# chasewalker26/Image-Classification-XAI

Measured on AMD Instinct MI355X. Metric: attributions/sec (IG 50-step ResNet-50 224^2), higher is better.
Workload: dtype f32

## Files before the change

image-classification-xai_amd/csrc/conv/conv1x1_bwd_wide_kernels.hip:

```cpp
#include "xai_common.h"
#include "xai_conv_walk.h"
#include "xai_convw.h"

XAI_VERSION_ENTRIES(xai_convw_version, XAI_CONVW_VERSION, XAI_CONVW_MINOR)

namespace {

typedef float f32x4 __attribute__((ext_vector_type(4)));

__device__ __forceinline__ f32x4 mfma4(float a, float b, f32x4 c) { return __builtin_amdgcn_mfma_f32_16x16x4f32(a, b, c, 0, 0, 0); }

__global__ __launch_bounds__(kWave) void conv1x1_bwd_wide_simple_kernel(const float* __restrict__ gy, const float* __restrict__ W, int K,
                                                                        int C, int HW, int grouping, int from_zero, XaiStagger st,
                                                                        float* __restrict__ gx) {
  const int lane = threadIdx.x, slot = lane >> 4, l16 = lane & 15;
  const int row = blockIdx.y * 16 + l16;
  const int col = blockIdx.x * 16 + l16;
  const bool row_ok = row < C, col_ok = col < HW;
  const float* gyn = gy + static_cast<int64_t>(blockIdx.z) * K * HW + (col_ok ? col : 0);
  float* gxn = gx + static_cast<int64_t>(blockIdx.z) * C * HW + (col_ok ? col : 0);
  const int first = xai_stagger_first(st, 16 * (st.axis == XAI_STAGGER_ROWS ? blockIdx.y : blockIdx.x));
  f32x4 acc = {0.f, 0.f, 0.f, 0.f};
  for (int t = 0; t < st.blocks; ++t) {
    const int k0 = xai_stagger_block(st, first, t) * kWalkBlock;
#pragma unroll
    for (int m = 0; m < 4; ++m) {
      const int k = k0 + xai_walk_k(grouping, m, slot);
      const float a = row_ok ? W[static_cast<int64_t>(k) * C + row] : 0.f;
      const float b = col_ok ? gyn[static_cast<int64_t>(k) * HW] : 0.f;
      acc = mfma4(a, b, acc);
    }
  }
  if (from_zero) acc = f32x4{0.f, 0.f, 0.f, 0.f} + acc;
  if (!col_ok) return;
#pragma unroll
  for (int r = 0; r < 4; ++r) {
    const int c = blockIdx.y * 16 + 4 * slot + r;
    if (c < C) gxn[static_cast<int64_t>(c) * HW] = acc[r];
  }
}

constexpr int kThreads = 256;
constexpr int kPad = 16;

__device__ __forceinline__ f32x4 load4(const float* p, int valid, bool vec) {
  f32x4 v = {0.f, 0.f, 0.f, 0.f};
  if (valid <= 0) return v;
  if (vec) return *reinterpret_cast<const f32x4*>(p);
#pragma unroll
  for (int j = 0; j < 4; ++j)
    if (j < valid) v[j] = p[j];
  return v;
}

template <int TM, int TN>
__global__ __launch_bounds__(kThreads) void conv1x1_bwd_wide_kernel(const float* __restrict__ gy, const float* __restrict__ W, int K, int C,
                                                                    int HW, int grouping, int from_zero, XaiStagger st, int hold, int vec,
                                                                    float* __restrict__ gx) {
  constexpr int LDA = TM + kPad, LDB = TN + kPad;
  constexpr int WROWS = TM / 32, WCOLS = 4 / WROWS, NJ = TN / (16 * WCOLS);
  constexpr int UA = TM / 4, UB = TN / 4;
  constexpr int RA = kWalkBlock * UA / kThreads;
  static_assert(RA >= 1 && kWalkBlock * UB <= kThreads && NJ >= 1, "tile sizes");
  extern __shared__ __attribute__((aligned(16))) float lds[];
  float* As = lds;
  float* Bs = lds + 2 * kWalkBlock * LDA;
  const int tid = threadIdx.x, lane = tid & (kWave - 1), wave = tid / kWave;
  const int slot = lane >> 4, l16 = lane & 15;
  const int col0 = blockIdx.x * TN, n = blockIdx.y;
  const int nb = st.blocks;
  const int chunks = hold ? (C + TM - 1) / TM : 1, chunk0 = hold ? 0 : blockIdx.z;
  const int first = xai_stagger_first(st, col0);

  const int bk = tid / UB, bj = (tid % UB) * 4;
  const bool b_lane = tid < kWalkBlock * UB;
  const int b_valid = b_lane ? min(4, HW - (col0 + bj)) : 0;
  const float* bp = gy + static_cast<int64_t>(n) * K * HW + (b_valid > 0 ? col0 + bj : 0);
  f32x4 ra[RA], rb;
  auto load = [&](int g) {
    const int chunk = chunk0 + g / nb, block = xai_stagger_block(st, first, g % nb);
    const int k0 = block * kWalkBlock;
#pragma unroll
    for (int r = 0; r < RA; ++r) {
      const int u = tid + r * kThreads, ak = u / UA, ai = chunk * TM + (u % UA) * 4;
      ra[r] = load4(W + static_cast<int64_t>(k0 + ak) * C + (ai < C ? ai : 0), C - ai, vec != 0);
    }
    if (g < nb || !hold) rb = load4(bp + static_cast<int64_t>(k0 + bk) * HW, b_valid, vec != 0);
  };
  auto stage = [&](int g) {
    float* A = As + (g & 1) * kWalkBlock * LDA;
#pragma unroll
    for (int r = 0; r < RA; ++r) {
      const int u = tid + r * kThreads, ak = u / UA, ai = (u % UA) * 4;
      *reinterpret_cast<f32x4*>(A + xai_walk_row(grouping, ak) * LDA + ai) = ra[r];
    }
    if (b_lane && (g < nb || !hold)) {
      float* B = Bs + (hold ? xai_stagger_block(st, first, g % nb) : (g & 1)) * kWalkBlock * LDB;
      *reinterpret_cast<f32x4*>(B + xai_walk_row(grouping, bk) * LDB + bj) = rb;
    }
  };

  const int wr = (wave / WCOLS) * 32, wc = (wave % WCOLS) * (16 * NJ);
  f32x4 acc[2][NJ];
#pragma unroll
  for (int i = 0; i < 2; ++i)
#pragma unroll
    for (int j = 0; j < NJ; ++j) acc[i][j] = f32x4{0.f, 0.f, 0.f, 0.f};

  const int slabs = chunks * nb;
  load(0);
  stage(0);
  __syncthreads();
  int t = 0;
  for (int g = 0; g < slabs; ++g) {
    const bool more = g + 1 < slabs;
    if (more) load(g + 1);
    const float* A = As + (g & 1) * kWalkBlock * LDA;
    const float* B = Bs + (hold ? xai_stagger_block(st, first, t) : (g & 1)) * kWalkBlock * LDB;
#pragma unroll
    for (int m = 0; m < 4; ++m) {
      const int krow = 4 * m + slot;
      const float a0 = A[krow * LDA + wr + l16], a1 = A[krow * LDA + wr + 16 + l16];
      float b[NJ];
#pragma unroll
      for (int j = 0; j < NJ; ++j) b[j] = B[krow * LDB + wc + 16 * j + l16];
#pragma unroll
      for (int j = 0; j < NJ; ++j) {
        acc[0][j] = mfma4(a0, b[j], acc[0][j]);
        acc[1][j] = mfma4(a1, b[j], acc[1][j]);
      }
    }
    if (more) stage(g + 1);
    __syncthreads();
    if (++t < nb) continue;
    t = 0;
    const int row0 = (chunk0 + g / nb) * TM;
#pragma unroll
    for (int j = 0; j < NJ; ++j) {
      const int col = col0 + wc + 16 * j + l16;
      float* out = gx + static_cast<int64_t>(n) * C * HW + col;
#pragma unroll
      for (int i = 0; i < 2; ++i) {
        if (from_zero) acc[i][j] = f32x4{0.f, 0.f, 0.f, 0.f} + acc[i][j];
#pragma unroll
        for (int r = 0; r < 4; ++r) {
          const int c = row0 + wr + 16 * i + 4 * slot + r;
          if (col < HW && c < C) out[static_cast<int64_t>(c) * HW] = acc[i][j][r];
        }
        acc[i][j] = f32x4{0.f, 0.f, 0.f, 0.f};
      }
    }
  }
}

constexpr int kHoldBytes = 40 * 1024;

static int wide_args_status(const float* gy, const float* weight, int N, int K, int C, int HW, int grouping, int depth, int tile, int axis,
                            int stagger, int stride, const float* gx, XaiStagger* st) {
  XAI_REQUIRE_PTR(gy); XAI_REQUIRE_PTR(weight); XAI_REQUIRE_PTR(gx);
  XAI_REQUIRE(N > 0 && K > 0 && C > 0 && HW > 0, XAI_E_SHAPE);
  XAI_REQUIRE(((reinterpret_cast<uintptr_t>(gy) | reinterpret_cast<uintptr_t>(weight) | reinterpret_cast<uintptr_t>(gx)) & 3u) == 0,
              XAI_E_SHAPE);
  XAI_REQUIRE(grouping == XAI_WALK_K_CONSECUTIVE || grouping == XAI_WALK_K_STRIDE4, XAI_E_SHAPE);
  XAI_REQUIRE(xai_stagger_plan(K, depth, tile, axis, stagger, stride, st), XAI_E_SHAPE);
  XAI_REQUIRE(N <= 65535 && static_cast<int64_t>(K) * HW <= INT32_MAX && static_cast<int64_t>(C) * HW <= INT32_MAX, XAI_E_UNSUPPORTED);
  return XAI_OK;
}

}

XAI_EXPORT int xai_convw_bwd_data_f32(const float* gy, const float* weight, int N, int K, int C, int HW, int grouping, int from_zero,
                                      int depth, int tile, int axis, int stagger, int stride, float* gx, xai_stream_t stream) {
  XaiStagger st;
  if (const int rc = wide_args_status(gy, weight, N, K, C, HW, grouping, depth, tile, axis, stagger, stride, gx, &st)) return rc;
  XAI_REQUIRE(st.mask == 0 || (axis == XAI_STAGGER_COLUMNS && tile % 32 == 0), XAI_E_UNSUPPORTED);
  const int tn = st.mask != 0 && tile % 64 != 0 ? 32 : 64, tm = C <= 64 ? 64 : 128;
  const int chunks = static_cast<int>(xai_ceil_div(C, tm));
  const size_t slab_b = sizeof(float) * kWalkBlock * (tn + kPad);
  const bool hold = chunks > 1 && slab_b * st.blocks <= static_cast<size_t>(kHoldBytes);
  XAI_REQUIRE(chunks <= 65535, XAI_E_UNSUPPORTED);
  const bool vec = HW % 4 == 0 && C % 4 == 0 && xai_aligned16(gy) && xai_aligned16(weight);
  const size_t lds = sizeof(float) * 2 * kWalkBlock * (tm + kPad) + slab_b * (hold ? st.blocks : 2);
  const dim3 grid(static_cast<unsigned>(xai_ceil_div(HW, tn)), static_cast<unsigned>(N), static_cast<unsigned>(hold ? 1 : chunks));
  hipStream_t s = static_cast<hipStream_t>(stream);
  xai_dispatch(tm == 128, [&](auto tall) {
    xai_dispatch(tn == 64, [&](auto broad) {
      constexpr int TM = decltype(tall)::value ? 128 : 64, TN = decltype(broad)::value ? 64 : 32;
      hipLaunchKernelGGL((conv1x1_bwd_wide_kernel<TM, TN>), grid, dim3(kThreads), lds, s, gy, weight, K, C, HW, grouping, from_zero != 0, st,
                         hold ? 1 : 0, vec ? 1 : 0, gx);
    });
  });
  return xai_launch_status();
}

XAI_EXPORT int xai_convw_bwd_data_simple_f32(const float* gy, const float* weight, int N, int K, int C, int HW, int grouping, int from_zero,
                                             int depth, int tile, int axis, int stagger, int stride, float* gx, xai_stream_t stream) {
  XaiStagger st;
  if (const int rc = wide_args_status(gy, weight, N, K, C, HW, grouping, depth, tile, axis, stagger, stride, gx, &st)) return rc;
  const dim3 grid(static_cast<unsigned>(xai_ceil_div(HW, 16)), static_cast<unsigned>(xai_ceil_div(C, 16)), static_cast<unsigned>(N));
  XAI_REQUIRE(grid.y <= 65535u, XAI_E_UNSUPPORTED);
  hipLaunchKernelGGL(conv1x1_bwd_wide_simple_kernel, grid, dim3(kWave), 0, static_cast<hipStream_t>(stream), gy, weight, K, C, HW, grouping,
                     from_zero != 0, st, gx);
  return xai_launch_status();
}
```

Measured before the change: 93.89.

## Deepen prefetch pipeline in wide 1x1 conv backward-data kernel and template on vector loads

Restructures the tiled MFMA kernel so that global loads run two slabs ahead, using two register sets, compile-time buffer parity, and incremental counters in place of per-iteration div/mod stagger recomputation. A sched_barrier pins the loads ahead of the MFMA loop, and the chunk loop is unrolled in pairs so buffer indices are constants. The vectorized-load flag becomes a template parameter, removing runtime branches, and the B-tile load is generalized to multiple rows per thread. The cost is higher register use, which may lower occupancy, plus more template instantiations. A benchmarking script is also added.

```diff
diff --git a/image-classification-xai_amd/csrc/conv/conv1x1_bwd_wide_kernels.hip b/image-classification-xai_amd/csrc/conv/conv1x1_bwd_wide_kernels.hip
--- a/image-classification-xai_amd/csrc/conv/conv1x1_bwd_wide_kernels.hip
+++ b/image-classification-xai_amd/csrc/conv/conv1x1_bwd_wide_kernels.hip
@@ -1,3 +1,5 @@
+#include <type_traits>
+
 #include "xai_common.h"
 #include "xai_conv_walk.h"
 #include "xai_convw.h"
@@ -43,25 +45,29 @@
 constexpr int kThreads = 256;
 constexpr int kPad = 16;
 
-__device__ __forceinline__ f32x4 load4(const float* p, int valid, bool vec) {
-  f32x4 v = {0.f, 0.f, 0.f, 0.f};
-  if (valid <= 0) return v;
-  if (vec) return *reinterpret_cast<const f32x4*>(p);
-#pragma unroll
-  for (int j = 0; j < 4; ++j)
-    if (j < valid) v[j] = p[j];
-  return v;
-}
-
-template <int TM, int TN>
+template <bool VEC>
+__device__ __forceinline__ f32x4 load4(const float* p, int valid) {
+  if constexpr (VEC) {
+    return *reinterpret_cast<const f32x4*>(p);
+  } else {
+    f32x4 v = {0.f, 0.f, 0.f, 0.f};
+#pragma unroll
+    for (int j = 0; j < 4; ++j)
+      if (j < valid) v[j] = p[j];
+    return v;
+  }
+}
+
+template <int TM, int TN, bool VEC>
 __global__ __launch_bounds__(kThreads) void conv1x1_bwd_wide_kernel(const float* __restrict__ gy, const float* __restrict__ W, int K, int C,
-                                                                    int HW, int grouping, int from_zero, XaiStagger st, int hold, int vec,
+                                                                    int HW, int grouping, int from_zero, XaiStagger st, int hold,
                                                                     float* __restrict__ gx) {
   constexpr int LDA = TM + kPad, LDB = TN + kPad;
   constexpr int WROWS = TM / 32, WCOLS = 4 / WROWS, NJ = TN / (16 * WCOLS);
   constexpr int UA = TM / 4, UB = TN / 4;
   constexpr int RA = kWalkBlock * UA / kThreads;
-  static_assert(RA >= 1 && kWalkBlock * UB <= kThreads && NJ >= 1, "tile sizes");
+  constexpr int RB = (kWalkBlock * UB + kThreads - 1) / kThreads;
+  static_assert(RA >= 1 && NJ >= 1 && TN % 16 == 0 && (RB == 1 || kWalkBlock * UB == RB * kThreads), "tile sizes");
   extern __shared__ __attribute__((aligned(16))) float lds[];
   float* As = lds;
   float* Bs = lds + 2 * kWalkBlock * LDA;
@@ -71,52 +77,72 @@
   const int nb = st.blocks;
   const int chunks = hold ? (C + TM - 1) / TM : 1, chunk0 = hold ? 0 : blockIdx.z;
   const int first = xai_stagger_first(st, col0);
-
-  const int bk = tid / UB, bj = (tid % UB) * 4;
-  const bool b_lane = tid < kWalkBlock * UB;
-  const int b_valid = b_lane ? min(4, HW - (col0 + bj)) : 0;
-  const float* bp = gy + static_cast<int64_t>(n) * K * HW + (b_valid > 0 ? col0 + bj : 0);
-  f32x4 ra[RA], rb;
-  auto load = [&](int g) {
-    const int chunk = chunk0 + g / nb, block = xai_stagger_block(st, first, g % nb);
-    const int k0 = block * kWalkBlock;
+  const int slabs = chunks * nb;
+
+  int64_t b_at[RB];
+  int bk[RB], bv[RB], b_valid[RB];
+#pragma unroll
+  for (int r = 0; r < RB; ++r) {
+    const int u = tid + r * kThreads, v = (u % UB) * 4, col = col0 + v;
+    const bool unit = u < kWalkBlock * UB;
+    bk[r] = unit ? u / UB : 0;
+    bv[r] = v;
+    b_valid[r] = unit ? min(4, HW - col) : 0;
+    b_at[r] = b_valid[r] > 0 ? static_cast<int64_t>(n) * K * HW + col : 0;
+  }
+  f32x4 ra[2][RA], rb[2][RB];
+  int l_n = 0, l_t = 0, l_chunk = chunk0, l_block = first;
+  int s_block[2] = {0, 0};
+  bool s_gy[2] = {false, false};
+  auto load = [&](auto set) {
+    constexpr int P = decltype(set)::value;
+    const bool live = l_n < slabs, gy_live = live && (!hold || l_chunk == chunk0);
+    const int k0 = live ? l_block * kWalkBlock : 0, chunk = live ? l_chunk : chunk0;
 #pragma unroll
     for (int r = 0; r < RA; ++r) {
       const int u = tid + r * kThreads, ak = u / UA, ai = chunk * TM + (u % UA) * 4;
-      ra[r] = load4(W + static_cast<int64_t>(k0 + ak) * C + (ai < C ? ai : 0), C - ai, vec != 0);
-    }
-    if (g < nb || !hold) rb = load4(bp + static_cast<int64_t>(k0 + bk) * HW, b_valid, vec != 0);
-  };
-  auto stage = [&](int g) {
-    float* A = As + (g & 1) * kWalkBlock * LDA;
+      const int64_t at = static_cast<int64_t>(k0 + ak) * C + (ai < C ? ai : 0);
+      ra[P][r] = load4<VEC>(W + (live ? at : 0), C - ai);
+    }
+#pragma unroll
+    for (int r = 0; r < RB; ++r) {
+      const int64_t at = b_at[r] + static_cast<int64_t>(k0 + bk[r]) * HW;
+      rb[P][r] = load4<VEC>(gy + (gy_live ? at : 0), gy_live ? b_valid[r] : 0);
+    }
+    s_block[P] = l_block;
+    s_gy[P] = gy_live;
+    ++l_n;
+    if (++l_block == nb) l_block = 0;
+    if (++l_t == nb) {
+      l_t = 0;
+      ++l_chunk;
+    }
+  };
+  auto stage = [&](auto set) {
+    constexpr int P = decltype(set)::value;
+    float* A = As + P * kWalkBlock * LDA;
 #pragma unroll
     for (int r = 0; r < RA; ++r) {
       const int u = tid + r * kThreads, ak = u / UA, ai = (u % UA) * 4;
-      *reinterpret_cast<f32x4*>(A + xai_walk_row(grouping, ak) * LDA + ai) = ra[r];
-    }
-    if (b_lane && (g < nb || !hold)) {
-      float* B = Bs + (hold ? xai_stagger_block(st, first, g % nb) : (g & 1)) * kWalkBlock * LDB;
-      *reinterpret_cast<f32x4*>(B + xai_walk_row(grouping, bk) * LDB + bj) = rb;
+      *reinterpret_cast<f32x4*>(A + xai_walk_row(grouping, ak) * LDA + ai) = ra[P][r];
+    }
+    if (s_gy[P]) {
+      float* B = Bs + (hold ? s_block[P] : P) * kWalkBlock * LDB;
+#pragma unroll
+      for (int r = 0; r < RB; ++r)
+        if (RB * kThreads == kWalkBlock * UB || tid < kWalkBlock * UB)
+          *reinterpret_cast<f32x4*>(B + xai_walk_row(grouping, bk[r]) * LDB + bv[r]) = rb[P][r];
     }
   };
 
   const int wr = (wave / WCOLS) * 32, wc = (wave % WCOLS) * (16 * NJ);
-  f32x4 acc[2][NJ];
-#pragma unroll
-  for (int i = 0; i < 2; ++i)
-#pragma unroll
-    for (int j = 0; j < NJ; ++j) acc[i][j] = f32x4{0.f, 0.f, 0.f, 0.f};
-
-  const int slabs = chunks * nb;
-  load(0);
-  stage(0);
-  __syncthreads();
-  int t = 0;
-  for (int g = 0; g < slabs; ++g) {
-    const bool more = g + 1 < slabs;
-    if (more) load(g + 1);
-    const float* A = As + (g & 1) * kWalkBlock * LDA;
-    const float* B = Bs + (hold ? xai_stagger_block(st, first, t) : (g & 1)) * kWalkBlock * LDB;
+  int g = 0, block = first;
+  auto step = [&](auto set, f32x4 (&acc)[2][NJ]) {
+    constexpr int P = decltype(set)::value;
+    load(set);
+    __builtin_amdgcn_sched_barrier(0);
+    const float* A = As + P * kWalkBlock * LDA;
+    const float* B = Bs + (hold ? block : P) * kWalkBlock * LDB;
 #pragma unroll
     for (int m = 0; m < 4; ++m) {
       const int krow = 4 * m + slot;
@@ -130,11 +156,24 @@
         acc[1][j] = mfma4(a1, b[j], acc[1][j]);
       }
     }
-    if (more) stage(g + 1);
+    if (g + 1 < slabs) stage(std::integral_constant<int, 1 - P>{});
     __syncthreads();
-    if (++t < nb) continue;
-    t = 0;
-    const int row0 = (chunk0 + g / nb) * TM;
+    ++g;
+    if (++block == nb) block = 0;
+  };
+  auto run_chunk = [&](auto set, int row0) {
+    constexpr int P = decltype(set)::value;
+    f32x4 acc[2][NJ];
+#pragma unroll
+    for (int i = 0; i < 2; ++i)
+#pragma unroll
+      for (int j = 0; j < NJ; ++j) acc[i][j] = f32x4{0.f, 0.f, 0.f, 0.f};
+    int t = 0;
+    for (; t + 1 < nb; t += 2) {
+      step(std::integral_constant<int, P>{}, acc);
+      step(std::integral_constant<int, 1 - P>{}, acc);
+    }
+    if (t < nb) step(std::integral_constant<int, P>{}, acc);
 #pragma unroll
     for (int j = 0; j < NJ; ++j) {
       const int col = col0 + wc + 16 * j + l16;
@@ -147,9 +186,19 @@
           const int c = row0 + wr + 16 * i + 4 * slot + r;
           if (col < HW && c < C) out[static_cast<int64_t>(c) * HW] = acc[i][j][r];
         }
-        acc[i][j] = f32x4{0.f, 0.f, 0.f, 0.f};
       }
     }
+  };
+
+  load(std::integral_constant<int, 0>{});
+  load(std::integral_constant<int, 1>{});
+  stage(std::integral_constant<int, 0>{});
+  __syncthreads();
+  int parity = 0;
+  for (int c = 0; c < chunks; ++c) {
+    if (parity) run_chunk(std::integral_constant<int, 1>{}, (chunk0 + c) * TM);
+    else run_chunk(std::integral_constant<int, 0>{}, (chunk0 + c) * TM);
+    parity ^= nb & 1;
   }
 }
 
@@ -185,9 +234,11 @@
   hipStream_t s = static_cast<hipStream_t>(stream);
   xai_dispatch(tm == 128, [&](auto tall) {
     xai_dispatch(tn == 64, [&](auto broad) {
-      constexpr int TM = decltype(tall)::value ? 128 : 64, TN = decltype(broad)::value ? 64 : 32;
-      hipLaunchKernelGGL((conv1x1_bwd_wide_kernel<TM, TN>), grid, dim3(kThreads), lds, s, gy, weight, K, C, HW, grouping, from_zero != 0, st,
-                         hold ? 1 : 0, vec ? 1 : 0, gx);
+      xai_dispatch(vec, [&](auto wide) {
+        constexpr int TM = decltype(tall)::value ? 128 : 64, TN = decltype(broad)::value ? 64 : 32;
+        hipLaunchKernelGGL((conv1x1_bwd_wide_kernel<TM, TN, decltype(wide)::value>), grid, dim3(kThreads), lds, s, gy, weight, K, C, HW,
+                           grouping, from_zero != 0, st, hold ? 1 : 0, gx);
+      });
     });
   });
   return xai_launch_status();
diff --git a/profiles/experiments/exp_k80_variants.py b/profiles/experiments/exp_k80_variants.py
--- /dev/null
+++ b/profiles/experiments/exp_k80_variants.py
@@ -0,0 +1,129 @@
+import ctypes
+import os
+import sys
+import threading
+import time
+
+HERE = os.path.dirname(os.path.abspath(__file__))
+sys.path.insert(0, os.path.join(os.path.dirname(os.path.dirname(HERE)), "image-classification-xai_amd"))
+sys.path.insert(0, HERE)
+import torch
+from exp_wide_bwd_which_kernels import MORE_SHAPES, SHAPES, operands
+from xai_engine import kernels as K
+from xai_engine import prepare, streams, zoo
+
+out = open(sys.argv[1], "w")
+variants = []
+for spec in sys.argv[2:]:
+    label, path = spec.split("=", 1)
+    fn = ctypes.CDLL(os.path.abspath(path)).xai_convw_bwd_data_f32
+    fn.argtypes = [ctypes.c_void_p] * 2 + [ctypes.c_int] * 11 + [ctypes.c_void_p] * 2
+    fn.restype = ctypes.c_int
+    variants.append((label, fn))
+
+
+def say(*a):
+    s = " ".join(str(v) for v in a)
+    print(s, flush=True)
+    out.write(s + "\n")
+    out.flush()
+
+
+def launch(fn, gy, weight, walk, gx):
+    N, Kc, H, W = gy.shape
+    rc = fn(gy.data_ptr(), weight.data_ptr(), N, Kc, weight.shape[1], H * W, *walk, gx.data_ptr(), torch.cuda.current_stream().cuda_stream)
+    assert rc == 0, rc
+
+
+def timed(f, reps=20):
+    for _ in range(3):
+        f()
+    a, b = torch.cuda.Event(enable_timing=True), torch.cuda.Event(enable_timing=True)
+    torch.cuda.current_stream().synchronize()
+    a.record()
+    for _ in range(reps):
+        f()
+    b.record()
+    torch.cuda.current_stream().synchronize()
+    return a.elapsed_time(b) / reps * 1e3
+
+
+torch.backends.cudnn.deterministic = True
+torch.backends.cudnn.benchmark = False
+dev = torch.device("cuda", 0)
+N = 50
+held = []
+g = torch.Generator(device="cuda").manual_seed(1)
+for label, Kc, Cc, H, W, folded in SHAPES + MORE_SHAPES:
+    if folded or H * W <= 64:
+        continue
+    x, y, gy, weight = operands(torch, g, Kc, Cc, H, W, folded, N)
+    (ref,) = torch.autograd.grad(y, x, gy, retain_graph=True)
+    walk = next((w for w in prepare._CONV_WIDE_WALKS
+                 if Kc % w[2] == 0 and bool((K.conv1x1_bwd_data_wide(gy, weight, w).view(torch.int32) == ref.view(torch.int32)).all())), None)
+    tag = f"{label} {Kc}->{Cc} on {H}x{W}"
+    if walk is None:
+        say(f"{tag}: no walk returns MIOpen's bits")
+        continue
+    same = []
+    for name, fn in variants:
+        buf = torch.full_like(ref, float("nan"))
+        launch(fn, gy, weight, walk, buf)
+        same.append(f"{name} {bool((buf.view(torch.int32) == ref.view(torch.int32)).all())}")
+    say(f"{tag}: walk {walk}; MIOpen's bits: " + ", ".join(same))
+    held.append((tag, (Kc, Cc, H, W, folded, N), walk))
+    del x, y, gy, ref
+
+model = zoo.resnet50().to(dev).eval()
+ws = streams.workers(dev, 3)
+stop = threading.Event()
+passes = [0, 0]
+
+
+def classifier_passes(i):
+    xin = torch.randn(50, 3, 224, 224, device=dev).requires_grad_(True)
+    last = None
+    while not stop.is_set():
+        torch.autograd.grad(model(xin).sum(), xin)
+        ev = torch.cuda.Event()
+        ev.record()
+        if last is not None:
+            last.synchronize()
+            passes[i] += 1
+        last = ev
+    torch.cuda.current_stream().synchronize()
+    return passes[i]
+
+
+def measure():
+    res, gen = [], torch.Generator(device="cuda").manual_seed(2)
+    for _, spec, w in held:
+        x, y, gy, weight = operands(torch, gen, *spec)
+        buf = torch.empty_like(x)
+        row = []
+        for _ in range(2):
+            row.append([timed(lambda: torch.autograd.grad(y, x, gy, retain_graph=True))]
+                       + [timed(lambda: launch(fn, gy, weight, w, buf)) for _, fn in variants])
+        res.append(row)
+        del x, y, gy, buf
+    return res
+
+
+alone = ws[2].submit(measure).result()
+busy = [ws[i].submit(lambda i=i: classifier_passes(i)) for i in (0, 1)]
+while min(passes) < 2 and not any(f.done() for f in busy):
+    time.sleep(0.05)
+before = list(passes)
+contended = ws[2].submit(measure).result()
+during = [b - a for a, b in zip(before, passes)]
+stop.set()
+for f in busy:
+    f.result()
+say(f"classifier passes finished by the two other streams during the contended measurement: {during}")
+names = ["MIOpen"] + [name for name, _ in variants]
+say("us per launch, two repeats each (MIOpen's with autograd's host overhead); columns: " + ", ".join(names))
+for (tag, _, w), a, c in zip(held, alone, contended):
+    say(f"{tag}:")
+    say("  alone  " + "  ".join(f"{n} {r0:6.1f} {r1:6.1f}" for n, r0, r1 in zip(names, a[0], a[1])))
+    say("  beside " + "  ".join(f"{n} {r0:6.1f} {r1:6.1f}" for n, r0, r1 in zip(names, c[0], c[1])))
+say("DONE")
```

Result: no change. 94.43 (median of 6 runs) (+0.6%).
